# koszullab/chromosight

Measured on AMD Instinct MI355X. Metric: Mpixels/s normxcorr2 (17x17 loops kernel), higher is better.
Workload: dtype f32

## Files before the change

### chromosight_amd/_lib.py

```python
import ctypes as C
import os
import pathlib
import threading
import weakref

import numpy as np

CS_F32, CS_F64 = 0, 1
LAYOUT_DENSE, LAYOUT_BAND, LAYOUT_BAND_LAZY, LAYOUT_BAND_PADDED, LAYOUT_BAND_COUNTS, LAYOUT_BAND_COUNTS_VIEW = 0, 1, 2, 3, 4, 5
COUNTS_HEADER_BYTES = 128
LAZY_BAND_BYTES = 128
MASK_NONE, MASK_BINS, MASK_EXPLICIT = 0, 1, 2

_LIB_PATH = pathlib.Path(os.environ.get("CHROMOSIGHT_HIP_LIBRARY") or pathlib.Path(__file__).with_name("libchromosight_hip.so"))


class CsMatrix(C.Structure):
    _fields_ = [
        ("d_ptr", C.c_void_p),
        ("dtype", C.c_int32),
        ("layout", C.c_int32),
        ("ld", C.c_int64),
        ("band_lo", C.c_int32),
        ("band_w", C.c_int32),
# ... 151 lines not shown
    CALL_ACCEPT_RECORDS, CALL_DETECT_FOCI_BATCH_FINISH, CALL_STREAM_WAIT_TILES = 1, 2, 3, 4, 5, 6, 7, 9

STAGE_SMOOTH = 1

CAPTURE = None
_CAPTURED = ("cs_stage_blocks", "cs_stage_blocks_opt", "cs_event_record", "cs_stream_wait_event", "cs_detect_foci_blocks", "cs_detect_foci_batch_templates")


FOCUS_DTYPE = np.dtype([("bin1", "<i4"), ("bin2", "<i4"), ("inside", "<i4"), ("n_zero", "<i4"), ("n_missing", "<i4"),
                        ("focus_size", "<i4"), ("score", "<f8"), ("n_obs", "<f8"), ("pval", "<f8")])


_PROTOTYPES = {
    "cs_version": (C.c_char_p, []),
    "cs_last_kernel": (C.c_int, [C.c_void_p]),
    "cs_ctx_set_range_check": (C.c_int, [C.c_void_p, C.c_int32]),
    "cs_ctx_create": (C.c_int, [C.c_int, C.POINTER(C.c_void_p)]),
    "cs_ctx_destroy": (None, [C.c_void_p]),
    "cs_last_error": (C.c_char_p, [C.c_void_p]),
    "cs_device_cu_count": (C.c_int, [C.c_void_p]),
    "cs_malloc": (C.c_int, [C.c_void_p, C.c_size_t, C.POINTER(C.c_void_p)]),
    "cs_free": (C.c_int, [C.c_void_p, C.c_void_p]),
    "cs_memcpy_h2d": (C.c_int, [C.c_void_p, C.c_void_p, C.c_void_p, C.c_size_t, C.c_void_p]),
    "cs_memcpy_d2h": (C.c_int, [C.c_void_p, C.c_void_p, C.c_void_p, C.c_size_t, C.c_void_p]),
    "cs_memset": (C.c_int, [C.c_void_p, C.c_void_p, C.c_int, C.c_size_t, C.c_void_p]),
    "cs_stream_sync": (C.c_int, [C.c_void_p, C.c_void_p]),
    "cs_stream_create": (C.c_int, [C.c_void_p, C.POINTER(C.c_void_p)]),
    "cs_stream_create_priority": (C.c_int, [C.c_void_p, C.c_int32, C.POINTER(C.c_void_p)]),
    "cs_stream_destroy": (C.c_int, [C.c_void_p, C.c_void_p]),
    "cs_event_create": (C.c_int, [C.c_void_p, C.POINTER(C.c_void_p)]),
# ... 350 lines not shown
```

### chromosight_amd/csrc/cs_api.cpp

```cpp
#include "cs_api_internal.h"

extern char** environ;

namespace csapi {

__global__ void cs_wait_tiles_kernel(const unsigned* word, unsigned epoch, long long ticks)
{
    const long long t0 = wall_clock64();
    while ((int)(__hip_atomic_load(word, __ATOMIC_RELAXED, __HIP_MEMORY_SCOPE_AGENT) - epoch) < 0 && wall_clock64() - t0 < ticks)
        __builtin_amdgcn_s_sleep(16);
}

int fail(cs_ctx* ctx, int code, const char* fmt, ...)
{
    if (ctx) {
        char buf[512];
        va_list ap;
        va_start(ap, fmt);
        vsnprintf(buf, sizeof(buf), fmt, ap);
        va_end(ap);
        ctx->err = buf;
    }
    return code;
}
// ... 390 lines not shown
    w.insert(w.end(), VB.begin(), VB.begin() + (size_t)rb * kn);
    w.insert(w.end(), (size_t)km, 1.0);
    w.insert(w.end(), UA.begin(), UA.begin() + (size_t)ra * km);
    w.insert(w.end(), UB.begin(), UB.begin() + (size_t)rb * km);
}

DispatchSwitches read_dispatch_switches()
{
    DispatchSwitches sw = {};
    sw.mfma = sw.mfma_reg = sw.large = sw.lowrank = -1;
    const struct { const char* name; bool* flag; int* digit; } known[] = {
        {"FORCE_GENERIC", &sw.force_generic, nullptr}, {"NO_MFMA", &sw.no_mfma, nullptr}, {"NO_WIDE", &sw.no_wide, nullptr},
        {"WIDE_ALL", &sw.wide_all, nullptr}, {"NO_LARGE", &sw.no_large, nullptr}, {"NO_SEPARABLE", &sw.no_separable, nullptr},
        {"SEPARABLE_FIRST", &sw.separable_first, nullptr}, {"NO_REGULAR_MASK", &sw.no_regular_mask, nullptr},
        {"FULL_MASK_TABLES", &sw.full_mask_tables, nullptr}, {"MFMA_NORSYM", &sw.mfma_norsym, nullptr},
        {"NO_SYMMETRY", &sw.no_symmetry, nullptr}, {"DEBUG", &sw.debug, nullptr}, {"MFMA", nullptr, &sw.mfma},
        {"MFMA_REG", nullptr, &sw.mfma_reg}, {"LARGE", nullptr, &sw.large}, {"LOWRANK", nullptr, &sw.lowrank},
    };
    constexpr size_t kPrefix = sizeof("CHROMOSIGHT_HIP_") - 1;
    for (char** e = environ; e && *e; ++e) {
        if ((*e)[0] != 'C' || std::strncmp(*e, "CHROMOSIGHT_HIP_", kPrefix) != 0) continue;
        const char* name = *e + kPrefix;
        const char* eq = std::strchr(name, '=');
        if (!eq) continue;
        for (const auto& k : known)
            if (std::strlen(k.name) == (size_t)(eq - name) && std::strncmp(k.name, name, eq - name) == 0) {
                if (k.flag) *k.flag = true;
                else *k.digit = eq[1] == '1' ? 1 : eq[1] == '0' ? 0 : -1;
            }
    }
    return sw;
// ... 265 lines not shown
    A.sig.ld = ld;
    A.sig.row0 = p_lo;
    A.sig_is_f64 = 0;
    return CS_OK;
}

static int run_lowrank(cs_ctx* ctx, cs::CorrArgs<float>& A, hipStream_t stream)
{
    const int rc = cs::launch_corr_lowrank_f32(A, stream);
    if (rc == cs::kLaunchNoFit || rc == cs::kLaunchNeedMap || rc == cs::kLaunchDeclined) return kNextRoute;
    if (rc != 0) return fail(ctx, CS_ERR_HIP, "kernel launch failed: %s", hipGetErrorString((hipError_t)rc));
    ctx->last_kernel = CS_KERNEL_LOWRANK;
    return CS_OK;
}

static int launch_tile_kernel(cs_ctx* ctx, cs::CorrArgs<float>& A, hipStream_t stream)
{
    cs::MfmaWeights E;
    int rc = ensure_wfrag(ctx, stream, A.km, A.kn, &E);
    if (rc != CS_OK) return rc;
    int path = 0;
    rc = cs::launch_corr_mfma_f32(A, E, stream, &path);
    ctx->last_kernel = path == 1 ? CS_KERNEL_MFMA_DENSE : path == 2 ? CS_KERNEL_MFMA_REG : path == 3 ? CS_KERNEL_MFMA_LIST : CS_KERNEL_MFMA;
    return rc;
}

static int run_mfma_reg(cs_ctx* ctx, cs::CorrArgs<float>& A, const DispatchSwitches& sw, hipStream_t stream)
{
    out_diagonals(A);
    if (A.cand_keys) {
        A.out_lo = std::max(A.out_lo, A.cand_dlo);
        A.out_hi = std::min(A.out_hi, A.cand_dhi);
    }
    int rc = prepare_regular_mask<float>(ctx, A, sw, A.km, stream, A.mfma_rsym != 0, true);
    if (rc != CS_OK) return rc;
    if (A.reg_mode != 1) return kNextRoute;
    if (A.sig_is_f64) {
        rc = narrow_f64_rows(ctx, A, A.sig.layout == CS_LAYOUT_BAND ? A.sig.band_w : A.ns, stream);
        if (rc != CS_OK) return rc;
    }
    rc = sink_result(ctx, launch_tile_kernel(ctx, A, stream));
    if (rc == CS_OK && (ctx->last_kernel == CS_KERNEL_MFMA_REG || ctx->last_kernel == CS_KERNEL_MFMA_LIST) && A.cand_keys) ctx->cand_fused = true;
    return rc;
}

static int run_mfma_wide(cs_ctx* ctx, cs::CorrArgs<float>& A, hipStream_t stream)
{
    cs::MfmaWideWeights E;
    int rc = ensure_wfrag_wide(ctx, stream, A.km, A.kn, &E);
    if (rc != CS_OK) return rc;
    const bool sink = !A.out.ptr;
    ctx->last_kernel = CS_KERNEL_MFMA_WIDE;
    rc = cs::launch_corr_mfma_wide_f32(A, E, stream);
    rc = sink ? sink_result(ctx, rc) : map_result(ctx, A.km, A.kn, rc);
    if (rc == CS_OK && sink) ctx->cand_fused = true;
    return rc;
}

static int run_mfma_large(cs_ctx* ctx, cs::CorrArgs<float>& A, hipStream_t stream)
{
    cs::MfmaLargeWeights E;
    int rc = ensure_wfrag_large(ctx, stream, A.km, A.kn, &E);
    if (rc != CS_OK) return rc;
    const bool sink = !A.out.ptr;
    ctx->last_kernel = CS_KERNEL_MFMA_LARGE;
    rc = sink_result(ctx, cs::launch_corr_mfma_large_f32(A, E, stream));
    if (rc == CS_OK && sink) ctx->cand_fused = true;
    return rc;
}

static int run_mfma(cs_ctx* ctx, cs::CorrArgs<float>& A, hipStream_t stream)
{
    if (A.sig_is_f64 && A.mask_mode == 0 && A.sig.layout == 0 && A.out.layout == 0 && !A.nobs.ptr) {
        const int rc = narrow_f64_rows(ctx, A, A.ns, stream);
        if (rc != CS_OK) return rc;
    }
    return map_result(ctx, A.km, A.kn, launch_tile_kernel(ctx, A, stream));
}

template <typename TC>
static int run_stream(cs_ctx* ctx, cs::CorrArgs<TC>& A, const DispatchSwitches& sw, hipStream_t stream)
{
    const FastKernel* f = fast_kernel(A.km, A.kn);
    int tw, th;
    ctx->last_kernel = CS_KERNEL_STREAM;
    f->tile(A.row_end - A.row_begin, A.ns, A.out.layout == 1 ? A.out.band_w : 0, ctx->n_cu, &tw, &th);
    fill_grid(A, tw, th, false);
    int rc = prepare_regular_mask<TC>(ctx, A, sw, f->K, stream);
    if (rc != CS_OK) return rc;
    if constexpr (sizeof(TC) == 4) rc = f->f32(A, stream);
    else rc = f->f64(A, stream);
    return map_result(ctx, A.km, A.kn, rc);
// ... 24 lines not shown
int launch_corr<float>(cs_ctx* ctx, cs::CorrArgs<float>& A, hipStream_t stream)
{
    const DispatchSwitches sw = read_dispatch_switches();
    const bool fast = !sw.force_generic;
    int rc;
    A.n_cu = ctx->n_cu;
    A.grid_cap = ctx->grid_cap;
    A.reg_mode = 0;
    A.mfma_rsym = A.w_sym && A.km == 17 && A.kn == 17 && !sw.mfma_norsym;
    if (fast && lowrank_wanted(A, sw) && (rc = run_lowrank(ctx, A, stream)) != kNextRoute) return rc;
    if (fast && mfma_reg_wanted(A, sw) && (rc = run_mfma_reg(ctx, A, sw, stream)) != kNextRoute) return rc;
    if (A.sig.counts) return fail(ctx, CS_ERR_UNSUPPORTED, "a band of counts (CS_LAYOUT_BAND_COUNTS) is read by the masked float32 tile kernel only: per-bin masks, full mode, odd square template of up to 17");
    if (fast && !A.out.ptr && mfma_wide_wanted(A, sw) && !A.w_rank1) return run_mfma_wide(ctx, A, stream);
    if (fast && mfma_large_wanted(A, sw)) return run_mfma_large(ctx, A, stream);
    if (!A.out.ptr) return CS_NEED_MAP;
    if (fast && mfma_wanted(A, sw)) return run_mfma(ctx, A, stream);
    if (fast && stream_wanted(A, sw)) return run_stream(ctx, A, sw, stream);
    if (fast && separable_wanted(A, sw)) return run_separable(ctx, A, stream);
    if (fast && mfma_wide_wanted(A, sw)) return run_mfma_wide(ctx, A, stream);
    return run_generic(ctx, A, stream);
}

template <>
int launch_corr<double>(cs_ctx* ctx, cs::CorrArgs<double>& A, hipStream_t stream)
{
    const DispatchSwitches sw = read_dispatch_switches();
    if (A.sig.counts) return fail(ctx, CS_ERR_UNSUPPORTED, "a band of counts (CS_LAYOUT_BAND_COUNTS) is read by the masked float32 tile kernel only");
    A.n_cu = ctx->n_cu;
    A.grid_cap = ctx->grid_cap;
    if (!sw.force_generic && stream_wanted(A, sw)) return run_stream(ctx, A, sw, stream);
    return run_generic(ctx, A, stream);
// ... 236 lines not shown
template int upload_weights<float>(cs_ctx*, hipStream_t, const std::vector<double>&);
template int upload_weights<double>(cs_ctx*, hipStream_t, const std::vector<double>&);
template int build_args<float>(cs_ctx*, hipStream_t, const cs_matrix*, const cs_kernel*, const cs_normxcorr2_params*, cs::CorrArgs<float>*);
template int build_args<double>(cs_ctx*, hipStream_t, const cs_matrix*, const cs_kernel*, const cs_normxcorr2_params*, cs::CorrArgs<double>*);

}

using namespace csapi;


extern "C" {

const char* cs_version(void) { return "chromosight_hip 0.1 (gfx950)"; }

int cs_last_kernel(const cs_ctx* ctx) { return ctx ? ctx->last_kernel : 0; }

int cs_ctx_set_range_check(cs_ctx* ctx, int32_t on)
{
    if (!ctx) return CS_ERR_INVALID;
    ctx->range_check = on ? 1 : 0;
    return CS_OK;
}

int cs_ctx_create(int device, cs_ctx** out)
{
    if (!out) return CS_ERR_INVALID;
    *out = nullptr;
    int count = 0;
    if (hipGetDeviceCount(&count) != hipSuccess || count <= 0) return CS_ERR_HIP;
    if (device < 0 || device >= count) return CS_ERR_INVALID;
// ... 199 lines not shown
```

### chromosight_amd/csrc/cs_api_internal.h

```cpp
#pragma once
#include <hip/hip_runtime.h>

#include <algorithm>
#include <mutex>
#include <memory>
#include <condition_variable>
#include <chrono>
#include <atomic>
#include <cmath>
#include <cstdarg>
#include <cstdio>
#include <cstdlib>
#include <cstring>
#include <limits>
#include <string>
#include <thread>
#include <unordered_map>
#include <type_traits>
#include <vector>

#include "../../include/chromosight_hip.h"
#include "cs_device.h"
#include "cs_launch.h"
#include "cs_launch_aux.h"
// ... 61 lines not shown
    int cand_n_tiles = 0;
    long long* h_cand_counts = nullptr;
    void* d_counts_peak = nullptr;
    unsigned* h_peak = nullptr;
    void* d_ws = nullptr;
    size_t d_ws_bytes = 0;
    WeightImage wfrag, wfrag_wide, wfrag_large;
    std::vector<cs::CorrArgs<double>> nb_tab;
    std::vector<long long> nb_seg;
    std::vector<int> nb_lo_w;
    int nb_pending = 0;
    long long nb_cap = 0;
    std::vector<char> stage_uploaded;
    void* d_rim = nullptr;
    int last_kernel = 0;
    int range_check = 0;
    bool cand_fused = false;
    long long cand_hint = 0, cand_hint_pixels = 0;
    int cand_hint_blocks = 0;
    bool cand_hint_paced = false;
    bool allow_lazy = false;
    bool allow_counts = false;
    long long uploads = 0;
    struct TemplateCache {
        std::vector<double> key;
        double stats[6] = {0, 0, 0, 0, 0, 0};
        std::vector<double> w;
        bool sym = false;
        bool rank1 = false;
        int lr = 0, lr2 = 0, lra = 0, lrb = 0;
// ... 164 lines not shown
extern template int upload_weights<float>(cs_ctx*, hipStream_t, const std::vector<double>&);
extern template int upload_weights<double>(cs_ctx*, hipStream_t, const std::vector<double>&);
int ensure_wfrag(cs_ctx* ctx, hipStream_t stream, int km, int kn, cs::MfmaWeights* E);
int factor_low_rank(const double* M, int km, int kn, int max_rank, std::vector<double>& U, std::vector<double>& V);
void append_lowrank_table(std::vector<double>& w, int km, int kn, const std::vector<double>& UA, const std::vector<double>& VA, int ra,
                          const std::vector<double>& UB, const std::vector<double>& VB, int rb);
constexpr int CS_NEED_MAP = 1000;
template <typename TC>
int launch_corr(cs_ctx* ctx, cs::CorrArgs<TC>& A, hipStream_t stream);
template <>
int launch_corr<float>(cs_ctx* ctx, cs::CorrArgs<float>& A, hipStream_t stream);
template <>
int launch_corr<double>(cs_ctx* ctx, cs::CorrArgs<double>& A, hipStream_t stream);
struct DispatchSwitches {
    bool force_generic, no_mfma, no_wide, wide_all, no_large, no_separable, separable_first, no_regular_mask, full_mask_tables,
        mfma_norsym, no_symmetry, debug;
    int mfma, mfma_reg, large, lowrank;
};
DispatchSwitches read_dispatch_switches();
template <typename TC>
int build_args(cs_ctx* ctx, hipStream_t stream, const cs_matrix* signal, const cs_kernel* kernel,
               const cs_normxcorr2_params* p, cs::CorrArgs<TC>* out);
extern template int build_args<float>(cs_ctx*, hipStream_t, const cs_matrix*, const cs_kernel*, const cs_normxcorr2_params*, cs::CorrArgs<float>*);
extern template int build_args<double>(cs_ctx*, hipStream_t, const cs_matrix*, const cs_kernel*, const cs_normxcorr2_params*, cs::CorrArgs<double>*);

}
```

### chromosight_amd/csrc/cs_corr_mfma.hip

```cpp
#include "cs_device.h"
#include <algorithm>
#include <cstdlib>
#include <cstring>
#include <mutex>
#include <utility>
#include <vector>

#include "cs_launch.h"

namespace cs {

typedef _Float16 h8 __attribute__((ext_vector_type(8)));

__device__ __forceinline__ float cand_range_guard(float r, float s2, float unscale, const KernelStats<float>& K);
typedef _Float16 h4 __attribute__((ext_vector_type(4)));
typedef float f4 __attribute__((ext_vector_type(4)));
typedef float f4u __attribute__((ext_vector_type(4), aligned(4)));
typedef double d2u __attribute__((ext_vector_type(2), aligned(8)));

constexpr int MF_T = 64;
constexpr int MF_R = 80;
constexpr int MF_PLANE = MF_R * MF_R * 2;
constexpr int MF_WSET = 17 * 2 * 1024;
constexpr int MF_SCR_PITCH = 40;
// ... 6 lines not shown
#ifdef CS_MF_DEBUG
#define MFD_DBG(bit) (A.dbg & (bit))
#else
#define MFD_DBG(bit) (false)
#endif

#ifdef CS_MF_PROFILE
__device__ unsigned long long cs_mf_prof[16];
#define MF_STAMP(k)                                                        \
    do {                                                                   \
        const unsigned long long now_ = __builtin_readcyclecounter();      \
        if (tid == 0) MF_PROF_ADD(k, now_ - tprev_);                       \
        tprev_ = now_;                                                     \
    } while (0)
#define MF_PROF_ADD(k, v) atomicAdd(&cs_mf_prof[k], (unsigned long long)(v))
#else
#define MF_STAMP(k)
#endif

__device__ __forceinline__ f4 mfma16(const h8& a, const h8& b, const f4& c)
{
    return __builtin_amdgcn_mfma_f32_16x16x32_f16(a, b, c, 0, 0, 0);
}

template <bool MASKED>
__global__ __launch_bounds__(256, 2) void corr_mfma_kernel(const CorrArgs<float> A, const MfmaWeights E)
{
    extern __shared__ __attribute__((aligned(16))) char smem[];
    _Float16* xh = reinterpret_cast<_Float16*>(smem);
    _Float16* xl = reinterpret_cast<_Float16*>(smem + MF_PLANE);
    _Float16* xm = reinterpret_cast<_Float16*>(smem + 2 * MF_PLANE);
    char* wreg = smem + 3 * MF_PLANE;
// ... 585 lines not shown
    bool ran = false;
    for (int b = 0; b < T.n_blocks; ++b) {
        const int s0 = first[b], s1 = first[b + 1];
        const int lo = max(lo_x, s0), hi = min(hi_x, s1);
        if (lo >= hi) continue;
        int g = lo_x + j;
        if (g < lo) g += (lo - g + step - 1) / step * step;
        if (g >= hi) continue;
        if (ran) lds_barrier();
        ran = true;
        const unsigned long long entry = (unsigned long long)(T.args + b);
        mfma_dense_tiles_table<true, true, RSYM, true>(*(MfmaDenseArgsC*)entry, entry, g - s0, hi - s0, step);
    }
}

static hipError_t allow_big_lds(const void* fn)
{
    static std::mutex mu;
    static std::vector<std::pair<const void*, int>> done;
    int dev = 0;
    hipError_t e = hipGetDevice(&dev);
    if (e != hipSuccess) return e;
    std::lock_guard<std::mutex> lock(mu);
    for (const auto& d : done)
        if (d.first == fn && d.second == dev) return hipSuccess;
    e = hipFuncSetAttribute(fn, hipFuncAttributeMaxDynamicSharedMemorySize, 160 * 1024);
    if (e == hipSuccess) done.emplace_back(fn, dev);
    return e;
}

// ... 9 lines not shown
            cols[n++] = (int)((t - by * tiles_x + by * s) % tiles_x);
        }
        for (int a = 0; a < n; ++a) {
            bool seen = false;
            for (int b = 0; b < a; ++b) seen |= cols[b] == cols[a];
            score += !seen;
        }
        if (score > best_score) {
            best_score = score;
            best = s;
        }
    }
    return best;
}

int launch_corr_mfma_f32(CorrArgs<float>& A, const MfmaWeights& E, hipStream_t stream, int* dense_path)
{
    *dense_path = 0;
    A.tile_w = A.tile_h = MF_T;
    A.tiles_y = (A.row_end - A.row_begin + MF_T - 1) / MF_T;
    if (A.out.layout == 1) {
        A.out_lo = A.out.band_lo;
        A.out_hi = A.out.band_lo + A.out.band_w - 1;
        A.tiles_x = (A.out.band_w + MF_T - 1 + MF_T - 1) / MF_T;
    } else {
        A.out_lo = -(1 << 30);
        A.out_hi = (1 << 30);
        A.tiles_x = (A.ns + MF_T - 1) / MF_T;
    }
    if (A.cand_keys) {
        A.out_lo = std::max(A.out_lo, A.cand_dlo);
        A.out_hi = std::min(A.out_hi, A.cand_dhi);
    }
// ... 126 lines not shown
            typedef void (*reg_kernel_t)(const MfmaDenseArgs);
            const reg_kernel_t kr = rsym ? (cand ? corr_mfma_dense_kernel<true, true, true, true> : corr_mfma_dense_kernel<true, true, true, false>)
                                         : (cand ? corr_mfma_dense_kernel<true, true, false, true> : corr_mfma_dense_kernel<true, true, false, false>);
            hipError_t e3 = allow_big_lds((const void*)kr);
            if (e3 != hipSuccess) return (int)e3;
            const int per_cu_r = 2;
            if (D.n_tiles <= 0) return 0;
            int grid_r = (int)std::min<long long>(D.n_tiles, (long long)per_cu_r * A.n_cu);
            if (A.grid_cap > 0 && grid_r > A.grid_cap) grid_r = std::max(8, A.grid_cap & ~7);
            hipLaunchKernelGGL(kr, dim3((unsigned)grid_r), dim3(256), MFD_SMEM_REG + MFD_LAUNCH_EXTRA, stream, D);
            return (int)hipGetLastError();
        }
        if (!A.out.ptr) return kLaunchNeedMap;
        const bool vec4 = ((uintptr_t)D.out % 32 == 0) && D.ld_out % 4 == 0 &&
                          ((A.kn - 1) / 2) % 4 == 0 && D.ns % 4 == 0 && D.ns >= 4 && !getenv("CHROMOSIGHT_HIP_MFMA_NOVEC");
        const void* kd = vec4 ? (const void*)corr_mfma_dense_kernel<true, false> : (const void*)corr_mfma_dense_kernel<false, false>;
        hipError_t e2 = allow_big_lds(kd);
        if (e2 != hipSuccess) return (int)e2;
        const int per_cu = 2;
        const int grid = (int)std::min<long long>(blocks, (long long)per_cu * A.n_cu);
        D.xcd_order |= dense_tile_skew(A.tiles_x, blocks, (D.xcd_order & 1) && grid % 8 == 0 ? grid / 8 : grid) << 1;
        if (vec4) hipLaunchKernelGGL((corr_mfma_dense_kernel<true, false>), dim3((unsigned)grid), dim3(256), (MFD_LAUNCH_EXTRA ? MFD_SMEM_REG + MFD_LAUNCH_EXTRA : MFD_SMEM), stream, D);
        else hipLaunchKernelGGL((corr_mfma_dense_kernel<false, false>), dim3((unsigned)grid), dim3(256), (MFD_LAUNCH_EXTRA ? MFD_SMEM_REG + MFD_LAUNCH_EXTRA : MFD_SMEM), stream, D);
        return (int)hipGetLastError();
    }
    if (A.sig.counts) return kLaunchDeclined;
    if (!A.out.ptr) return kLaunchNeedMap;
    const void* kern = masked ? (const void*)corr_mfma_kernel<true> : (const void*)corr_mfma_kernel<false>;
    hipError_t e = allow_big_lds(kern);
    if (e != hipSuccess) return (int)e;
    if (masked) hipLaunchKernelGGL(corr_mfma_kernel<true>, dim3((unsigned)blocks), dim3(256), MF_SMEM, stream, A, E);
    else hipLaunchKernelGGL(corr_mfma_kernel<false>, dim3((unsigned)blocks), dim3(256), MF_SMEM, stream, A, E);
    return (int)hipGetLastError();
}

size_t mfma_blocks_arg_bytes() { return sizeof(MfmaDenseArgs); }
// ... 64 lines not shown
```

### chromosight_amd/csrc/cs_corr_mfma_body.inc

```

    extern __shared__ __attribute__((aligned(16))) char smem[];
    char* const pl_xh = smem;
    char* const pl_xl = smem + MF_PLANE;
    char* const pl_qh = smem + 2 * MF_PLANE;
    char* const pl_ql = smem + 3 * MF_PLANE;
    float* const raw = reinterpret_cast<float*>(smem + 2 * MF_PLANE);
    const int tid = threadIdx.x;
    const int lane = tid & 63, wv = tid >> 6;
    const int n = lane & 15, g = lane >> 4;
    char* const scr = smem + MFD_SCR + wv * (2 * MF_SCR_PLANE);
    unsigned* const red = reinterpret_cast<unsigned*>(smem + MFD_RED);
    const int km = A.km, kn = A.kn;
    const int kh = (km - 1) / 2, kw = (kn - 1) / 2;
#ifdef CS_MF_PROFILE
#undef MF_PROF_ADD
#define MF_PROF_ADD(k, v) (prof_lds[k] += (unsigned long long)(v))
    unsigned long long* const prof_lds = reinterpret_cast<unsigned long long*>(smem + MFD_PROF);
    unsigned long long tprev_ = 0;
    if (tid == 0)
        for (int k = 0; k < 16; ++k) prof_lds[k] = 0;
    auto prof_flush = [&]() {
        if (tid == 0)
            for (int k = 0; k < 16; ++k)
                if (prof_lds[k]) atomicAdd(&cs_mf_prof[k], prof_lds[k]);
    };
#endif

    h8 ones_b, ones_p;
#pragma unroll
    for (int e = 0; e < 8; ++e) {
        const int t = 8 * g + e - n;
        ones_b[e] = (t >= 0 && t < kn) ? (_Float16)1.0f : (_Float16)0.0f;
        const int rho = (e < 4 ? 4 * g + e : 16 + 4 * g + (e - 4)) - n;
        ones_p[e] = (rho >= 0 && rho < km) ? (_Float16)1.0f : (_Float16)0.0f;
    }
    const f4 zero4 = {0.0f, 0.0f, 0.0f, 0.0f};
// ... 669 lines not shown
#pragma unroll
        for (int k = 0; k < 5; ++k) {
            const int idx = min(tid + 256 * k, kSlots * 64 - 1);
            const int slot = idx >> 6;
            const int row = RSYM ? (slot < 9 ? slot : slot - 9) : slot, part = RSYM ? (slot < 9 ? 1 : 0) : 1;
            tails[k] = frag[(2 * min(row, km - 1) + part) * 64 + (idx & 63)];
        }
#pragma unroll
        for (int k = 0; k < 5; ++k) {
            const int idx = tid + 256 * k;
            const int slot = idx >> 6;
            const int row = RSYM ? (slot < 9 ? slot : slot - 9) : slot;
            if (idx < kSlots * 64) reinterpret_cast<h8*>(smem + MFD_WL)[idx] = row < km ? tails[k] : z;
        }
    }
    for (;; tile += tile_step) {
        const bool have = REG ? tile < tile_end : true;
        if constexpr (REG) {
            if (!have && !pending) break;
        } else {
            if (tile >= tile_end) break;
        }
        int I0 = 0, J0 = 0;
        if (have) tile_origin(tile, I0, J0);
        const int P0 = I0 - kh, Q0 = J0 - kw;
        bool inside = P0 >= p_min && P0 + MF_R - 1 <= p_max && Q0 >= 0 && Q0 + MF_R <= A.ns;
        if (REG && A.band_in) inside = inside && Q0 - (P0 + MF_R - 1) - A.lo_in >= 0 && Q0 + MF_R - 1 - P0 - A.lo_in <= A.bw_in - 1;
        if (REG && VEC4) inside = inside || (P0 >= pad_row0 && P0 + MF_R - 1 <= p_max);
        if (REG && MFD_DBG(512)) inside = true;
        if MFD_DBG(1024) {
// ... 327 lines not shown
        MF_STAMP(4);
#pragma unroll
        for (int c = 0; c < 4; ++c) {
            p_acc[c] = acc[c];
            p_S1[c] = S1[c];
            p_S2[c] = S2[c];
        }
        p_I0 = I0;
        p_J0 = J0;
        p_unscale = unscale;
        p_slot = slot;
        if constexpr (REG) p_hdr = *reinterpret_cast<const f4*>(A.rowtab + 4 * (size_t)min(I0 + wr0 + n, A.ms - 1));
        slot ^= 1;
        pending = true;
    }
    if constexpr (!REG) {
        if (pending) emit(p_I0, p_J0, p_unscale, p_acc, p_S1, p_S2, p_hdr, p_slot);
    }
#ifdef CS_MF_PROFILE
    prof_flush();
#undef MF_PROF_ADD
#define MF_PROF_ADD(k, v) atomicAdd(&cs_mf_prof[k], (unsigned long long)(v))
#endif
```

### chromosight_amd/csrc/cs_launch.h

```cpp
#pragma once
#include "cs_device.h"

namespace cs {

enum LaunchStatus : int {
    kLaunchNoFit = -3,
    kLaunchNarrowRows = -4,
    kLaunchNeedMap = -5,
    kLaunchDeclined = -6,
};

#define CS_DECL_FAST(K)                                                        \
    int launch_corr_fast_f32_k##K(const CorrArgs<float>& A, hipStream_t s);    \
    int launch_corr_fast_f64_k##K(const CorrArgs<double>& A, hipStream_t s);   \
    void corr_fast_tile_k##K(int ms, int ns, int band_w, int n_cu, int* tw, int* th);
CS_DECL_FAST(7)
CS_DECL_FAST(9)
CS_DECL_FAST(11)
CS_DECL_FAST(13)
CS_DECL_FAST(15)
CS_DECL_FAST(17)
#undef CS_DECL_FAST

int launch_corr_generic_f32(const CorrArgs<float>& A, hipStream_t s);
int launch_corr_generic_f64(const CorrArgs<double>& A, hipStream_t s);
void corr_generic_tile(int km, int kn, int* tw, int* th);
int launch_corr_sep_f32(const CorrArgs<float>& A, hipStream_t s);
bool corr_sep_fits(int km, int kn, bool masked);
void corr_sep_tile(int* tw, int* th);
bool corr_lowrank_supports(const CorrArgs<float>& A);
int launch_corr_lowrank_f32(const CorrArgs<float>& A, hipStream_t s);

struct MfmaWeights {
    const uint4* frag;
    float unscale[3];
    const float* rim;
};
constexpr int kRimPW = 0, kRimQW = 2 * 17 * 18, kRimW = 4 * 17 * 18, kRimBase = 4 * 17 * 18 + 2 * 289;
constexpr int kRimFloats = kRimBase + 3 * 17;
int launch_corr_mfma_f32(CorrArgs<float>& A, const MfmaWeights& E, hipStream_t s, int* dense_path);
size_t mfma_blocks_arg_bytes();
size_t mfma_blocks_arg_offset(int n_blocks);
size_t mfma_blocks_table_bytes(int n_blocks);
int mfma_blocks_table_finish(void* h_table, int n_blocks);
int launch_corr_mfma_blocks(void* h_table, void* d_table, int n_blocks, int rsym, int n_cu, hipStream_t s, hipStream_t upload, bool do_upload, bool launch,
                            unsigned* started = nullptr, unsigned epoch = 0);
int launch_corr_mfma_prepared(const void* h_arg, int rsym, int n_cu, int grid_cap, hipStream_t s);

struct MfmaWideWeights {
    const uint4* frag;
    float unscale[3];
    const float* sums;
    int plane_only;
    int plane_only_staging;
    int one_launch;
// ... 16 lines not shown
```

### include/chromosight_hip.h

```cpp
#ifndef CHROMOSIGHT_HIP_H
#define CHROMOSIGHT_HIP_H

#include <stddef.h>
#include <stdint.h>

#ifdef __cplusplus
extern "C" {
#endif

typedef struct cs_ctx cs_ctx;

typedef enum {
    CS_OK = 0,
    CS_ERR_INVALID = -1,
    CS_ERR_HIP = -2,
    CS_ERR_UNSUPPORTED = -3,
    CS_ERR_OVERFLOW = -4,
    CS_ERR_RANGE = -5
} cs_status;

enum { CS_F32 = 0, CS_F64 = 1, CS_U8 = 2  };
enum { CS_LAYOUT_DENSE = 0, CS_LAYOUT_BAND = 1, CS_LAYOUT_BAND_LAZY = 2 ,
       CS_LAYOUT_BAND_PADDED = 3,
       CS_LAYOUT_BAND_COUNTS = 4,
       CS_LAYOUT_BAND_COUNTS_VIEW = 5 };
#define CS_COUNTS_HEADER_BYTES 128
#define CS_COUNTS_LAW_BYTES(n, n_diags) (8ll * (2 * (int64_t)(n_diags) + 2) + 4ll * (((int64_t)(n_diags) + 3) / 2 * 2) + 4ll * (int64_t)(n))
enum { CS_MASK_NONE = 0, CS_MASK_BINS = 1, CS_MASK_EXPLICIT = 2 };

int cs_ctx_create(int device, cs_ctx** out);
void cs_ctx_destroy(cs_ctx* ctx);
const char* cs_last_error(const cs_ctx* ctx);
int cs_device_cu_count(const cs_ctx* ctx);
const char* cs_version(void);
enum { CS_KERNEL_NONE = 0, CS_KERNEL_GENERIC = 1, CS_KERNEL_STREAM = 2, CS_KERNEL_MFMA = 3, CS_KERNEL_MFMA_DENSE = 4,
       CS_KERNEL_MFMA_REG = 5, CS_KERNEL_SEPARABLE = 6, CS_KERNEL_MFMA_WIDE = 7, CS_KERNEL_MFMA_LIST = 8,
       CS_KERNEL_MFMA_LARGE = 9, CS_KERNEL_LOWRANK = 10 };
int cs_last_kernel(const cs_ctx* ctx);
int cs_ctx_set_range_check(cs_ctx* ctx, int32_t on);

int cs_malloc(cs_ctx* ctx, size_t bytes, void** d_ptr);
int cs_free(cs_ctx* ctx, void* d_ptr);
int cs_memcpy_h2d(cs_ctx* ctx, void* d_dst, const void* h_src, size_t bytes, void* stream);
int cs_memcpy_d2h(cs_ctx* ctx, void* h_dst, const void* d_src, size_t bytes, void* stream);
int cs_memset(cs_ctx* ctx, void* d_dst, int value, size_t bytes, void* stream);
int cs_stream_sync(cs_ctx* ctx, void* stream);
int cs_stream_create(cs_ctx* ctx, void** stream);
int cs_stream_create_priority(cs_ctx* ctx, int32_t high, void** stream);
int cs_stream_destroy(cs_ctx* ctx, void* stream);
int cs_event_create(cs_ctx* ctx, void** event);
int cs_event_destroy(cs_ctx* ctx, void* event);
int cs_event_record(cs_ctx* ctx, void* event, void* stream);
int cs_stream_wait_event(cs_ctx* ctx, void* stream, void* event);
// ... 257 lines not shown
```

Before: 203,400.

## Add 8-wave dense MFMA kernel specialized for 17x17 symmetric templates

```diff
diff --git a/chromosight_amd/_lib.py b/chromosight_amd/_lib.py
--- a/chromosight_amd/_lib.py
+++ b/chromosight_amd/_lib.py
@@ -189,6 +189,7 @@
 _PROTOTYPES = {
     "cs_version": (C.c_char_p, []),
     "cs_last_kernel": (C.c_int, [C.c_void_p]),
+    "cs_last_dense_waves": (C.c_int, [C.c_void_p]),
     "cs_ctx_set_range_check": (C.c_int, [C.c_void_p, C.c_int32]),
     "cs_ctx_create": (C.c_int, [C.c_int, C.POINTER(C.c_void_p)]),
     "cs_ctx_destroy": (None, [C.c_void_p]),
diff --git a/chromosight_amd/csrc/cs_api.cpp b/chromosight_amd/csrc/cs_api.cpp
--- a/chromosight_amd/csrc/cs_api.cpp
+++ b/chromosight_amd/csrc/cs_api.cpp
@@ -428,7 +428,7 @@
         {"WIDE_ALL", &sw.wide_all, nullptr}, {"NO_LARGE", &sw.no_large, nullptr}, {"NO_SEPARABLE", &sw.no_separable, nullptr},
         {"SEPARABLE_FIRST", &sw.separable_first, nullptr}, {"NO_REGULAR_MASK", &sw.no_regular_mask, nullptr},
         {"FULL_MASK_TABLES", &sw.full_mask_tables, nullptr}, {"MFMA_NORSYM", &sw.mfma_norsym, nullptr},
-        {"NO_SYMMETRY", &sw.no_symmetry, nullptr}, {"DEBUG", &sw.debug, nullptr}, {"MFMA", nullptr, &sw.mfma},
+        {"NO_SYMMETRY", &sw.no_symmetry, nullptr}, {"DEBUG", &sw.debug, nullptr}, {"MFMA_WAVES4", &sw.mfma_waves4, nullptr}, {"MFMA", nullptr, &sw.mfma},
         {"MFMA_REG", nullptr, &sw.mfma_reg}, {"LARGE", nullptr, &sw.large}, {"LOWRANK", nullptr, &sw.lowrank},
     };
     constexpr size_t kPrefix = sizeof("CHROMOSIGHT_HIP_") - 1;
@@ -724,13 +724,14 @@
     return CS_OK;
 }
 
-static int launch_tile_kernel(cs_ctx* ctx, cs::CorrArgs<float>& A, hipStream_t stream)
+static int launch_tile_kernel(cs_ctx* ctx, cs::CorrArgs<float>& A, const DispatchSwitches& sw, hipStream_t stream)
 {
     cs::MfmaWeights E;
+    ctx->last_dense_waves = 0;
     int rc = ensure_wfrag(ctx, stream, A.km, A.kn, &E);
     if (rc != CS_OK) return rc;
     int path = 0;
-    rc = cs::launch_corr_mfma_f32(A, E, stream, &path);
+    rc = cs::launch_corr_mfma_f32(A, E, stream, &path, sw.mfma_waves4, &ctx->last_dense_waves);
     ctx->last_kernel = path == 1 ? CS_KERNEL_MFMA_DENSE : path == 2 ? CS_KERNEL_MFMA_REG : path == 3 ? CS_KERNEL_MFMA_LIST : CS_KERNEL_MFMA;
     return rc;
 }
@@ -749,7 +750,7 @@
         rc = narrow_f64_rows(ctx, A, A.sig.layout == CS_LAYOUT_BAND ? A.sig.band_w : A.ns, stream);
         if (rc != CS_OK) return rc;
     }
-    rc = sink_result(ctx, launch_tile_kernel(ctx, A, stream));
+    rc = sink_result(ctx, launch_tile_kernel(ctx, A, sw, stream));
     if (rc == CS_OK && (ctx->last_kernel == CS_KERNEL_MFMA_REG || ctx->last_kernel == CS_KERNEL_MFMA_LIST) && A.cand_keys) ctx->cand_fused = true;
     return rc;
 }
@@ -779,13 +780,13 @@
     return rc;
 }
 
-static int run_mfma(cs_ctx* ctx, cs::CorrArgs<float>& A, hipStream_t stream)
+static int run_mfma(cs_ctx* ctx, cs::CorrArgs<float>& A, const DispatchSwitches& sw, hipStream_t stream)
 {
     if (A.sig_is_f64 && A.mask_mode == 0 && A.sig.layout == 0 && A.out.layout == 0 && !A.nobs.ptr) {
         const int rc = narrow_f64_rows(ctx, A, A.ns, stream);
         if (rc != CS_OK) return rc;
     }
-    return map_result(ctx, A.km, A.kn, launch_tile_kernel(ctx, A, stream));
+    return map_result(ctx, A.km, A.kn, launch_tile_kernel(ctx, A, sw, stream));
 }
 
 template <typename TC>
@@ -840,7 +841,7 @@
     if (fast && !A.out.ptr && mfma_wide_wanted(A, sw) && !A.w_rank1) return run_mfma_wide(ctx, A, stream);
     if (fast && mfma_large_wanted(A, sw)) return run_mfma_large(ctx, A, stream);
     if (!A.out.ptr) return CS_NEED_MAP;
-    if (fast && mfma_wanted(A, sw)) return run_mfma(ctx, A, stream);
+    if (fast && mfma_wanted(A, sw)) return run_mfma(ctx, A, sw, stream);
     if (fast && stream_wanted(A, sw)) return run_stream(ctx, A, sw, stream);
     if (fast && separable_wanted(A, sw)) return run_separable(ctx, A, stream);
     if (fast && mfma_wide_wanted(A, sw)) return run_mfma_wide(ctx, A, stream);
@@ -1107,6 +1108,7 @@
 const char* cs_version(void) { return "chromosight_hip 0.1 (gfx950)"; }
 
 int cs_last_kernel(const cs_ctx* ctx) { return ctx ? ctx->last_kernel : 0; }
+int cs_last_dense_waves(const cs_ctx* ctx) { return ctx && ctx->last_kernel == CS_KERNEL_MFMA_DENSE ? ctx->last_dense_waves : 0; }
 
 int cs_ctx_set_range_check(cs_ctx* ctx, int32_t on)
 {
diff --git a/chromosight_amd/csrc/cs_api_internal.h b/chromosight_amd/csrc/cs_api_internal.h
--- a/chromosight_amd/csrc/cs_api_internal.h
+++ b/chromosight_amd/csrc/cs_api_internal.h
@@ -99,6 +99,7 @@
     std::vector<char> stage_uploaded;
     void* d_rim = nullptr;
     int last_kernel = 0;
+    int last_dense_waves = 0;
     int range_check = 0;
     bool cand_fused = false;
     long long cand_hint = 0, cand_hint_pixels = 0;
@@ -293,7 +294,7 @@
 int launch_corr<double>(cs_ctx* ctx, cs::CorrArgs<double>& A, hipStream_t stream);
 struct DispatchSwitches {
     bool force_generic, no_mfma, no_wide, wide_all, no_large, no_separable, separable_first, no_regular_mask, full_mask_tables,
-        mfma_norsym, no_symmetry, debug;
+        mfma_norsym, no_symmetry, debug, mfma_waves4;
     int mfma, mfma_reg, large, lowrank;
 };
 DispatchSwitches read_dispatch_switches();
diff --git a/chromosight_amd/csrc/cs_corr_mfma.hip b/chromosight_amd/csrc/cs_corr_mfma.hip
--- a/chromosight_amd/csrc/cs_corr_mfma.hip
+++ b/chromosight_amd/csrc/cs_corr_mfma.hip
@@ -44,8 +44,15 @@
         tprev_ = now_;                                                     \
     } while (0)
 #define MF_PROF_ADD(k, v) atomicAdd(&cs_mf_prof[k], (unsigned long long)(v))
+#define MF_WALL(k)                                                           \
+    do {                                                                     \
+        const unsigned long long w_ = __builtin_amdgcn_s_memrealtime();      \
+        if (tid == 0) prof_lds[k] += w_ - wall_;                             \
+        wall_ = w_;                                                          \
+    } while (0)
 #else
 #define MF_STAMP(k)
+#define MF_WALL(k)
 #endif
 
 __device__ __forceinline__ f4 mfma16(const h8& a, const h8& b, const f4& c)
@@ -661,6 +668,8 @@
     }
 }
 
+#include "cs_corr_mfma_dense8.inc"
+
 static hipError_t allow_big_lds(const void* fn)
 {
     static std::mutex mu;
@@ -700,9 +709,10 @@
     return best;
 }
 
-int launch_corr_mfma_f32(CorrArgs<float>& A, const MfmaWeights& E, hipStream_t stream, int* dense_path)
+int launch_corr_mfma_f32(CorrArgs<float>& A, const MfmaWeights& E, hipStream_t stream, int* dense_path, bool waves4, int* dense_waves)
 {
     *dense_path = 0;
+    if (dense_waves) *dense_waves = 0;
     A.tile_w = A.tile_h = MF_T;
     A.tiles_y = (A.row_end - A.row_begin + MF_T - 1) / MF_T;
     if (A.out.layout == 1) {
@@ -859,12 +869,19 @@
         if (!A.out.ptr) return kLaunchNeedMap;
         const bool vec4 = ((uintptr_t)D.out % 32 == 0) && D.ld_out % 4 == 0 &&
                           ((A.kn - 1) / 2) % 4 == 0 && D.ns % 4 == 0 && D.ns >= 4 && !getenv("CHROMOSIGHT_HIP_MFMA_NOVEC");
-        const void* kd = vec4 ? (const void*)corr_mfma_dense_kernel<true, false> : (const void*)corr_mfma_dense_kernel<false, false>;
+        const bool waves8 = vec4 && A.mfma_rsym != 0 && A.km == 17 && A.kn == 17 && !waves4;
+        const void* kd = waves8 ? (const void*)corr_mfma_dense8_kernel
+                         : vec4 ? (const void*)corr_mfma_dense_kernel<true, false> : (const void*)corr_mfma_dense_kernel<false, false>;
         hipError_t e2 = allow_big_lds(kd);
         if (e2 != hipSuccess) return (int)e2;
         const int per_cu = 2;
         const int grid = (int)std::min<long long>(blocks, (long long)per_cu * A.n_cu);
         D.xcd_order |= dense_tile_skew(A.tiles_x, blocks, (D.xcd_order & 1) && grid % 8 == 0 ? grid / 8 : grid) << 1;
+        if (dense_waves) *dense_waves = waves8 ? 8 : 4;
+        if (waves8) {
+            hipLaunchKernelGGL(corr_mfma_dense8_kernel, dim3((unsigned)grid), dim3(512), MF8_LAUNCH, stream, D);
+            return (int)hipGetLastError();
+        }
         if (vec4) hipLaunchKernelGGL((corr_mfma_dense_kernel<true, false>), dim3((unsigned)grid), dim3(256), (MFD_LAUNCH_EXTRA ? MFD_SMEM_REG + MFD_LAUNCH_EXTRA : MFD_SMEM), stream, D);
         else hipLaunchKernelGGL((corr_mfma_dense_kernel<false, false>), dim3((unsigned)grid), dim3(256), (MFD_LAUNCH_EXTRA ? MFD_SMEM_REG + MFD_LAUNCH_EXTRA : MFD_SMEM), stream, D);
         return (int)hipGetLastError();
diff --git a/chromosight_amd/csrc/cs_corr_mfma_body.inc b/chromosight_amd/csrc/cs_corr_mfma_body.inc
--- a/chromosight_amd/csrc/cs_corr_mfma_body.inc
+++ b/chromosight_amd/csrc/cs_corr_mfma_body.inc
@@ -17,9 +17,11 @@
 #define MF_PROF_ADD(k, v) (prof_lds[k] += (unsigned long long)(v))
     unsigned long long* const prof_lds = reinterpret_cast<unsigned long long*>(smem + MFD_PROF);
     unsigned long long tprev_ = 0;
+    unsigned long long wall_ = __builtin_amdgcn_s_memrealtime();
     if (tid == 0)
         for (int k = 0; k < 16; ++k) prof_lds[k] = 0;
     auto prof_flush = [&]() {
+        if (tid == 0) prof_lds[5] += 1ull;
         if (tid == 0)
             for (int k = 0; k < 16; ++k)
                 if (prof_lds[k]) atomicAdd(&cs_mf_prof[k], prof_lds[k]);
@@ -719,6 +721,7 @@
             if (idx < kSlots * 64) reinterpret_cast<h8*>(smem + MFD_WL)[idx] = row < km ? tails[k] : z;
         }
     }
+    MF_WALL(12);
     for (;; tile += tile_step) {
         const bool have = REG ? tile < tile_end : true;
         if constexpr (REG) {
@@ -1076,9 +1079,11 @@
         slot ^= 1;
         pending = true;
     }
+    MF_WALL(13);
     if constexpr (!REG) {
         if (pending) emit(p_I0, p_J0, p_unscale, p_acc, p_S1, p_S2, p_hdr, p_slot);
     }
+    MF_WALL(14);
 #ifdef CS_MF_PROFILE
     prof_flush();
 #undef MF_PROF_ADD
diff --git a/chromosight_amd/csrc/cs_corr_mfma_dense8.inc b/chromosight_amd/csrc/cs_corr_mfma_dense8.inc
--- /dev/null
+++ b/chromosight_amd/csrc/cs_corr_mfma_dense8.inc
@@ -0,0 +1,430 @@
+
+constexpr int MF8_ROWS_PER_THREAD = 7;
+constexpr int MF8_RED = MFD_WL + 18 * 1024;
+constexpr int MF8_SMEM = MF8_RED + 64;
+#ifdef CS_MF_PROFILE
+constexpr int MF8_PROF = MF8_SMEM;
+constexpr int MF8_LAUNCH = MF8_SMEM + 128;
+#else
+constexpr int MF8_LAUNCH = MF8_SMEM;
+#endif
+static_assert(MF8_LAUNCH <= 80 * 1024, "two workgroups per CU");
+
+__global__ __launch_bounds__(512, 4) void corr_mfma_dense8_kernel(const MfmaDenseArgs A)
+{
+    extern __shared__ __attribute__((aligned(16))) char smem[];
+    typedef __attribute__((address_space(3))) char lds_char;
+    char* const pl_xh = smem;
+    char* const pl_xl = smem + MF_PLANE;
+    char* const pl_qh = smem + 2 * MF_PLANE;
+    char* const pl_ql = smem + 3 * MF_PLANE;
+    float* const raw = reinterpret_cast<float*>(smem + 2 * MF_PLANE);
+    unsigned* const red = reinterpret_cast<unsigned*>(smem + MF8_RED);
+    const int tid = threadIdx.x;
+    const int lane = tid & 63, wv = tid >> 6;
+    const int n = lane & 15, g = lane >> 4;
+    constexpr int K = 17, KH = 8;
+#ifdef CS_MF_PROFILE
+#undef MF_PROF_ADD
+#define MF_PROF_ADD(k, v) (prof_lds[k] += (unsigned long long)(v))
+    unsigned long long* const prof_lds = reinterpret_cast<unsigned long long*>(smem + MF8_PROF);
+    unsigned long long tprev_ = 0;
+    unsigned long long wall_ = __builtin_amdgcn_s_memrealtime();
+    if (tid == 0)
+        for (int k = 0; k < 16; ++k) prof_lds[k] = 0;
+#endif
+
+    h8 ones_b, ones_p;
+#pragma unroll
+    for (int e = 0; e < 8; ++e) {
+        const int t = 8 * g + e - n;
+        ones_b[e] = (t >= 0 && t < K) ? (_Float16)1.0f : (_Float16)0.0f;
+        const int rho = (e < 4 ? 4 * g + e : 16 + 4 * g + (e - 4)) - n;
+        ones_p[e] = (rho >= 0 && rho < K) ? (_Float16)1.0f : (_Float16)0.0f;
+    }
+    const f4 zero4 = {0.0f, 0.0f, 0.0f, 0.0f};
+    const int wr0 = 16 * (wv & 3), wc0 = 32 * (wv >> 2);
+    const int c2 = tid % 40, rg = tid / 40;
+    const bool stager = tid < 480;
+    const int p_min = max(0, A.row_begin - KH), p_max = min(A.ms, A.row_end + (K - 1) - KH) - 1;
+
+    auto tile_origin = [&](int tile, int& I0, int& J0) {
+        const int by = tile / A.tiles_x;
+        int bx = tile - by * A.tiles_x;
+        const int skew = A.xcd_order >> 1;
+        if (skew) {
+            bx += (by * skew) % A.tiles_x;
+            bx -= bx >= A.tiles_x ? A.tiles_x : 0;
+        }
+        I0 = A.row_begin + by * MF_T;
+        J0 = bx * MF_T;
+    };
+    const int wv_u = __builtin_amdgcn_readfirstlane(wv);
+    auto fetch = [&](int tile) {
+        int I0, J0;
+        tile_origin(tile, I0, J0);
+        const int P0 = I0 - KH, Q0 = J0 - KH;
+        const int e0 = 64 * wv_u + lane;
+        int r = e0 / 20, c = e0 - r * 20;
+        const lds_char* dst = (const lds_char*)(raw) + 1024 * wv_u;
+        if (P0 >= p_min && P0 + MF_R - 1 <= p_max && Q0 >= 0 && Q0 + MF_R <= A.ns) {
+            const float* src = A.sig + ((long long)P0 + r - A.row0_in) * A.ld_in + Q0 + 4 * c;
+            const long long step_r = 25 * A.ld_in + 48, wrap = A.ld_in - 80;
+#pragma unroll 1
+            for (int i = wv_u; i < 25; i += 8) {
+                __builtin_amdgcn_global_load_lds(src, (__attribute__((address_space(3))) void*)dst, 16, 0, 0);
+                dst += 8192;
+                c += 12;
+                src += step_r;
+                if (c >= 20) {
+                    c -= 20;
+                    src += wrap;
+                }
+            }
+            return;
+        }
+#pragma unroll 1
+        for (int i = wv_u; i < 25; i += 8) {
+            const int p = min(max(P0 + r, p_min), p_max);
+            const int q = min(max(Q0 + 4 * c, 0), A.ns - 4);
+            const float* src = A.sig + ((long long)p - A.row0_in) * A.ld_in + q;
+            __builtin_amdgcn_global_load_lds(src, (__attribute__((address_space(3))) void*)dst, 16, 0, 0);
+            dst += 8192;
+            c += 12;
+            r += 25;
+            if (c >= 20) {
+                c -= 20;
+                r += 1;
+            }
+        }
+    };
+
+    auto emit = [&](int I0, int J0, float unscale, const f4 (&acc)[2], const f4 (&S1)[2], const f4 (&S2)[2]) {
+        const float u_cs = unscale * A.w_unscale;
+        const float u_s2 = 32.0f * unscale;
+        const bool plain = I0 + MF_T <= A.row_end && J0 + MF_T <= A.ns &&
+                           (A.full || (I0 >= KH && I0 + MF_T - 1 <= A.ms - K + KH && J0 >= KH && J0 + MF_T - 1 <= A.ns - K + KH)) &&
+                           (!A.sym_upper || J0 - (I0 + MF_T - 1) >= 0);
+        const int i = I0 + wr0 + n;
+        f4 rv[2];
+        bool lean = !A.xcorr_only && !(A.ks.cand_cmin > 0.0f);
+        if (lean) {
+            const KernelStats<float>& KS = A.ks;
+            const float inv_u = __uint_as_float((254u << 23) - __float_as_uint(unscale));
+            const float t1 = KS.thr_n * inv_u;
+            const float t2 = (t1 * inv_u) * 0.03125f;
+            const float td = (KS.den2_min * inv_u) * inv_u;
+            const float top = (fmaxf(KS.kvar, 1.0f) * 4294967296.0f) * (unscale * unscale);
+            auto normal_or_0 = [](float x) { return x == 0.0f || (x >= 1.17549435e-38f && x <= 3.40282347e38f); };
+            lean = normal_or_0(t1) && normal_or_0(t2) && normal_or_0(td) && td > 0.0f && top <= 3.40282347e38f;
+            if (lean) {
+                const float n32 = 32.0f * KS.n, wu = A.w_unscale;
+                bool normal = true;
+#pragma unroll
+                for (int c = 0; c < 2; ++c) {
+#pragma unroll
+                    for (int v = 0; v < 4; ++v) {
+                        const float s1 = S1[c][v], s2 = S2[c][v], cw = acc[c][v] * wu;
+                        const float den2 = fmaf(s2, n32, -s1 * s1) * KS.kvar;
+                        float r = cw * __builtin_amdgcn_rsqf(den2);
+                        r = (den2 >= td) ? r : 0.0f;
+                        rv[c][v] = __builtin_amdgcn_fmed3f(r, -1.0f, 1.0f);
+                        normal &= (int)(fabsf(s1) >= t1) & (int)(s2 >= t2) & (int)(fabsf(fmaf(KS.kmean, s1, cw)) >= t1);
+                    }
+                }
+                lean = !__builtin_amdgcn_ballot_w64(!normal);
+            }
+        }
+        if (!lean)
+#pragma unroll
+        for (int c = 0; c < 2; ++c) {
+#pragma unroll
+            for (int v = 0; v < 4; ++v) {
+                const float cs = acc[c][v] * u_cs;
+                const float s1 = S1[c][v] * unscale;
+                const float s2 = (S2[c][v] * u_s2) * unscale;
+                rv[c][v] = A.xcorr_only ? (fabsf(cs) < A.ks.thr ? 0.0f : cs)
+                                        : cand_range_guard(pearson_nomask_lean(cs, s1, s2, A.ks), s2, unscale, A.ks);
+            }
+        }
+        if (plain) {
+            const bool top8 = n < 8;
+            f4 s0, s1;
+#pragma unroll
+            for (int v = 0; v < 4; ++v) {
+                const float mine = top8 ? rv[1][v] : rv[0][v];
+                const float theirs = __builtin_bit_cast(float, __builtin_amdgcn_update_dpp(0, __builtin_bit_cast(int, mine), 0x128, 0xf, 0xf, true));
+                s0[v] = top8 ? rv[0][v] : theirs;
+                s1[v] = top8 ? theirs : rv[1][v];
+            }
+            const long long r_idx = ((long long)(I0 + wr0 + (n & 7)) - A.row0_out) * A.ld_out + J0 + wc0 + (top8 ? 0 : 16) + 4 * g;
+            if (A.out_is_f64) {
+                typedef double d2 __attribute__((ext_vector_type(2)));
+                double* od = reinterpret_cast<double*>(A.out) + r_idx;
+                d2 a, b;
+                a[0] = s0[0]; a[1] = s0[1]; b[0] = s0[2]; b[1] = s0[3];
+                *reinterpret_cast<d2*>(od) = a;
+                *reinterpret_cast<d2*>(od + 2) = b;
+                a[0] = s1[0]; a[1] = s1[1]; b[0] = s1[2]; b[1] = s1[3];
+                *reinterpret_cast<d2*>(od + 8 * A.ld_out) = a;
+                *reinterpret_cast<d2*>(od + 8 * A.ld_out + 2) = b;
+            } else {
+                float* of = reinterpret_cast<float*>(A.out) + r_idx;
+                *reinterpret_cast<f4*>(of) = s0;
+                *reinterpret_cast<f4*>(of + 8 * A.ld_out) = s1;
+            }
+        } else {
+            const long long o_idx = ((long long)i - A.row0_out) * A.ld_out + (J0 + wc0 + 4 * g);
+#pragma unroll
+            for (int c = 0; c < 2; ++c) {
+#pragma unroll
+                for (int v = 0; v < 4; ++v) {
+                    const int j = J0 + wc0 + 16 * c + 4 * g + v;
+                    bool z = false;
+                    if (!A.full) z = (i < KH) | (i > A.ms - K + KH) | (j < KH) | (j > A.ns - K + KH);
+                    if (A.sym_upper) z = z | ((j - i) < 0);
+                    if (i < A.row_end && j < A.ns) {
+                        const float val = z ? 0.0f : rv[c][v];
+                        if (A.out_is_f64) reinterpret_cast<double*>(A.out)[o_idx + 16 * c + v] = (double)val;
+                        else reinterpret_cast<float*>(A.out)[o_idx + 16 * c + v] = val;
+                    }
+                }
+            }
+        }
+    };
+
+    f4 p_acc[2], p_S1[2], p_S2[2];
+    int p_I0 = 0, p_J0 = 0;
+    float p_unscale = 0.0f;
+    bool pending = false;
+#pragma unroll
+    for (int c = 0; c < 2; ++c) p_acc[c] = p_S1[c] = p_S2[c] = zero4;
+
+    int tile, tile_end, tile_step;
+    if ((A.xcd_order & 1) && gridDim.x % 8 == 0) {
+        const int x = blockIdx.x & 7, per = (A.n_tiles + 7) / 8;
+        tile = x * per + (blockIdx.x >> 3);
+        tile_end = min(A.n_tiles, (x + 1) * per);
+        tile_step = gridDim.x >> 3;
+    } else {
+        tile = blockIdx.x;
+        tile_end = A.n_tiles;
+        tile_step = gridDim.x;
+    }
+    if (tile < tile_end) fetch(tile);
+
+    {
+        const h8* frag = reinterpret_cast<const h8*>(A.frag);
+        h8 wf[3];
+#pragma unroll
+        for (int k = 0; k < 3; ++k) {
+            const int idx = min(tid + 512 * k, 18 * 64 - 1);
+            const int slot = idx >> 6;
+            const int row = slot < 9 ? slot : slot - 9, part = slot < 9 ? 1 : 0;
+            wf[k] = frag[(2 * row + part) * 64 + (idx & 63)];
+        }
+#pragma unroll
+        for (int k = 0; k < 3; ++k) {
+            const int idx = tid + 512 * k;
+            if (idx < 18 * 64) reinterpret_cast<h8*>(smem + MFD_WL)[idx] = wf[k];
+        }
+    }
+    MF_WALL(12);
+    for (; tile < tile_end; tile += tile_step) {
+        int I0, J0;
+        tile_origin(tile, I0, J0);
+        const int P0 = I0 - KH, Q0 = J0 - KH;
+        const bool inside = P0 >= p_min && P0 + MF_R - 1 <= p_max && Q0 >= 0 && Q0 + MF_R <= A.ns;
+#ifdef CS_MF_PROFILE
+        tprev_ = __builtin_readcyclecounter();
+        if (tid == 0) prof_lds[15] += 1ull;
+#endif
+        __builtin_amdgcn_s_waitcnt(0x0f70);
+        lds_barrier();
+        float xa[MF8_ROWS_PER_THREAD], xb[MF8_ROWS_PER_THREAD];
+        float amax = 0.0f;
+        if (inside) {
+#pragma unroll
+            for (int k = 0; k < MF8_ROWS_PER_THREAD; ++k) {
+                const int r = rg + 12 * k;
+                float2 v = make_float2(0.0f, 0.0f);
+                if (stager && r < MF_R) v = *reinterpret_cast<const float2*>(raw + r * MF_R + 2 * c2);
+                xa[k] = v.x;
+                xb[k] = v.y;
+                amax = fmaxf(amax, fmaxf(fabsf(v.x), fabsf(v.y)));
+            }
+        } else {
+#pragma unroll
+            for (int k = 0; k < MF8_ROWS_PER_THREAD; ++k) {
+                const int r = rg + 12 * k;
+                float a = 0.0f, b = 0.0f;
+                if (stager && r < MF_R) {
+                    const float2 v = *reinterpret_cast<const float2*>(raw + r * MF_R + 2 * c2);
+                    const int p = P0 + r, q = Q0 + 2 * c2;
+                    const bool rok = (p >= p_min) & (p <= p_max);
+                    const bool oka = rok & (q >= 0) & (q < A.ns), okb = rok & (q + 1 >= 0) & (q + 1 < A.ns);
+                    a = oka ? v.x : 0.0f;
+                    b = okb ? v.y : 0.0f;
+                }
+                xa[k] = a;
+                xb[k] = b;
+                amax = fmaxf(amax, fmaxf(fabsf(a), fabsf(b)));
+            }
+        }
+        amax = wave_max_nonneg(amax);
+        if (lane == 63) red[wv] = __float_as_uint(amax);
+        MF_STAMP(0);
+        lds_barrier();
+        int ex = 0;
+        {
+            const uint4 m4 = *reinterpret_cast<const uint4*>(red), m8 = *reinterpret_cast<const uint4*>(red + 4);
+            const unsigned mx = max(max(max(m4.x, m4.y), max(m4.z, m4.w)), max(max(m8.x, m8.y), max(m8.z, m8.w)));
+            const int e = (int)((mx >> 23) & 0xffu);
+            if (e != 0 && e != 255) ex = 6 - (e - 127);
+            ex = max(-100, min(100, ex));
+        }
+        const float scale = __uint_as_float((unsigned)(ex + 127) << 23);
+        const float qscale = __uint_as_float((unsigned)(ex + 127 - 5) << 23);
+        const float unscale = __uint_as_float((unsigned)(127 - ex) << 23);
+        typedef __fp16 hv2 __attribute__((ext_vector_type(2)));
+#pragma unroll
+        for (int k = 0; k < MF8_ROWS_PER_THREAD; ++k) {
+            const int r = rg + 12 * k;
+            if (stager && r < MF_R) {
+                const float a = xa[k] * scale, b = xb[k] * scale;
+                const hv2 hh = __builtin_amdgcn_cvt_pkrtz(a, b);
+                const float qa = (xa[k] * qscale) * a, qb = (xb[k] * qscale) * b;
+                const hv2 qh = __builtin_amdgcn_cvt_pkrtz(qa, qb);
+                const unsigned hu = __builtin_bit_cast(unsigned, hh), qu = __builtin_bit_cast(unsigned, qh);
+                const hv2 tt = __builtin_amdgcn_cvt_pkrtz(sub_f16_lo(a, hu), sub_f16_hi(b, hu));
+                const hv2 qt = __builtin_amdgcn_cvt_pkrtz(sub_f16_lo(qa, qu), sub_f16_hi(qb, qu));
+                const int o = (r * MF_R + 2 * c2) * 2;
+                *reinterpret_cast<hv2*>(pl_xh + o) = hh;
+                *reinterpret_cast<hv2*>(pl_xl + o) = tt;
+                *reinterpret_cast<hv2*>(pl_qh + o) = qh;
+                *reinterpret_cast<hv2*>(pl_ql + o) = qt;
+            }
+        }
+        MF_STAMP(1);
+        if (pending) emit(p_I0, p_J0, p_unscale, p_acc, p_S1, p_S2);
+        MF_STAMP(6);
+        lds_barrier();
+
+        f4 S1[2], S2[2];
+#pragma unroll
+        for (int c = 0; c < 2; ++c) S1[c] = S2[c] = zero4;
+        if (!A.xcorr_only) {
+            auto hfrag = [&](int t, h8 (&f)[4]) {
+                const int c = t >> 1;
+                const char* ph = (t & 1) ? pl_qh : pl_xh;
+                const char* pt = (t & 1) ? pl_ql : pl_xl;
+#pragma unroll
+                for (int rb = 0; rb < 2; ++rb) {
+                    const int off = ((wr0 + 16 * rb + n) * MF_R + wc0 + 16 * c + 8 * g) * 2;
+                    f[2 * rb] = *reinterpret_cast<const h8*>(ph + off);
+                    f[2 * rb + 1] = *reinterpret_cast<const h8*>(pt + off);
+                }
+            };
+            h8 cur[4];
+            hfrag(0, cur);
+#pragma unroll
+            for (int t = 0; t < 4; ++t) {
+                h8 nxt[4];
+                if (t + 1 < 4) hfrag(t + 1, nxt);
+                typedef unsigned u4 __attribute__((ext_vector_type(4)));
+                u4 bhw, blw;
+#pragma unroll
+                for (int rb = 0; rb < 2; ++rb) {
+                    f4 h = mfma16(cur[2 * rb], ones_b, zero4);
+                    h = mfma16(cur[2 * rb + 1], ones_b, h);
+#pragma unroll
+                    for (int pr = 0; pr < 2; ++pr) {
+                        const unsigned hp = pack_h2((_Float16)h[2 * pr], (_Float16)h[2 * pr + 1]);
+                        bhw[2 * rb + pr] = hp;
+                        blw[2 * rb + pr] = pack_h2((_Float16)sub_f16_lo(h[2 * pr], hp), (_Float16)sub_f16_hi(h[2 * pr + 1], hp));
+                    }
+                }
+                const h8 bh = __builtin_bit_cast(h8, bhw), bl = __builtin_bit_cast(h8, blw);
+                f4 sacc = mfma16(bh, ones_p, zero4);
+                sacc = mfma16(bl, ones_p, sacc);
+                if (t & 1) S2[t >> 1] = sacc;
+                else S1[t >> 1] = sacc;
+                if (t + 1 < 4) {
+#pragma unroll
+                    for (int q = 0; q < 4; ++q) cur[q] = nxt[q];
+                }
+            }
+        }
+        MF_STAMP(2);
+        lds_barrier();
+        if (tile + tile_step < tile_end) fetch(tile + tile_step);
+
+        MF_STAMP(3);
+        f4 acc[2];
+#pragma unroll
+        for (int c = 0; c < 2; ++c) acc[c] = zero4;
+        h8 ah[2], al[2];
+        const int fo = ((wr0 + n) * MF_R + wc0 + 8 * g) * 2;
+#pragma unroll
+        for (int c = 0; c < 2; ++c) {
+            ah[c] = *reinterpret_cast<const h8*>(pl_xh + fo + 32 * c);
+            al[c] = *reinterpret_cast<const h8*>(pl_xl + fo + 32 * c);
+        }
+        h8 bl = reinterpret_cast<const h8*>(smem + MFD_WL)[lane];
+        h8 bh = reinterpret_cast<const h8*>(smem + MFD_WL)[9 * 64 + lane];
+#pragma unroll
+        for (int s = 0; s < 17; ++s) {
+            h8 nh[2], nl[2], nb, nbh;
+            if (s + 1 < 17) {
+#pragma unroll
+                for (int c = 0; c < 2; ++c) {
+                    nh[c] = *reinterpret_cast<const h8*>(pl_xh + fo + (s + 1) * MF_R * 2 + 32 * c);
+                    nl[c] = *reinterpret_cast<const h8*>(pl_xl + fo + (s + 1) * MF_R * 2 + 32 * c);
+                }
+                const int sn = s + 1 > 8 ? 16 - (s + 1) : s + 1;
+                nb = reinterpret_cast<const h8*>(smem + MFD_WL)[sn * 64 + lane];
+                nbh = reinterpret_cast<const h8*>(smem + MFD_WL)[(9 + sn) * 64 + lane];
+            }
+            __builtin_amdgcn_sched_barrier(0);
+#pragma unroll
+            for (int c = 0; c < 2; ++c) acc[c] = mfma16(bh, ah[c], acc[c]);
+#pragma unroll
+            for (int c = 0; c < 2; ++c) acc[c] = mfma16(bl, ah[c], acc[c]);
+#pragma unroll
+            for (int c = 0; c < 2; ++c) acc[c] = mfma16(bh, al[c], acc[c]);
+            __builtin_amdgcn_sched_barrier(0);
+            if (s + 1 < 17) {
+#pragma unroll
+                for (int c = 0; c < 2; ++c) {
+                    ah[c] = nh[c];
+                    al[c] = nl[c];
+                }
+                bl = nb;
+                bh = nbh;
+            }
+        }
+        MF_STAMP(4);
+#pragma unroll
+        for (int c = 0; c < 2; ++c) {
+            p_acc[c] = acc[c];
+            p_S1[c] = S1[c];
+            p_S2[c] = S2[c];
+        }
+        p_I0 = I0;
+        p_J0 = J0;
+        p_unscale = unscale;
+        pending = true;
+    }
+    MF_WALL(13);
+    if (pending) emit(p_I0, p_J0, p_unscale, p_acc, p_S1, p_S2);
+    MF_WALL(14);
+#ifdef CS_MF_PROFILE
+    if (tid == 0) {
+        prof_lds[5] += 1ull;
+        for (int k = 0; k < 16; ++k)
+            if (prof_lds[k]) atomicAdd(&cs_mf_prof[k], prof_lds[k]);
+    }
+#undef MF_PROF_ADD
+#define MF_PROF_ADD(k, v) atomicAdd(&cs_mf_prof[k], (unsigned long long)(v))
+#endif
+}
diff --git a/chromosight_amd/csrc/cs_launch.h b/chromosight_amd/csrc/cs_launch.h
--- a/chromosight_amd/csrc/cs_launch.h
+++ b/chromosight_amd/csrc/cs_launch.h
@@ -38,7 +38,7 @@
 };
 constexpr int kRimPW = 0, kRimQW = 2 * 17 * 18, kRimW = 4 * 17 * 18, kRimBase = 4 * 17 * 18 + 2 * 289;
 constexpr int kRimFloats = kRimBase + 3 * 17;
-int launch_corr_mfma_f32(CorrArgs<float>& A, const MfmaWeights& E, hipStream_t s, int* dense_path);
+int launch_corr_mfma_f32(CorrArgs<float>& A, const MfmaWeights& E, hipStream_t s, int* dense_path, bool waves4 = false, int* dense_waves = nullptr);
 size_t mfma_blocks_arg_bytes();
 size_t mfma_blocks_arg_offset(int n_blocks);
 size_t mfma_blocks_table_bytes(int n_blocks);
diff --git a/include/chromosight_hip.h b/include/chromosight_hip.h
--- a/include/chromosight_hip.h
+++ b/include/chromosight_hip.h
@@ -37,6 +37,7 @@
        CS_KERNEL_MFMA_REG = 5, CS_KERNEL_SEPARABLE = 6, CS_KERNEL_MFMA_WIDE = 7, CS_KERNEL_MFMA_LIST = 8,
        CS_KERNEL_MFMA_LARGE = 9, CS_KERNEL_LOWRANK = 10 };
 int cs_last_kernel(const cs_ctx* ctx);
+int cs_last_dense_waves(const cs_ctx* ctx);
 int cs_ctx_set_range_check(cs_ctx* ctx, int32_t on);
 
 int cs_malloc(cs_ctx* ctx, size_t bytes, void** d_ptr);
```

Measured after the change: 227,300, median of 6. 11.8% higher.
